# redwarp/kmeans-gpu

Hardware: AMD Instinct MI355X
Metric: pixels/sec per Lloyd iteration (8192x8192, k=256) (higher is better)
Workload: dtype f32; 1 GPU; synthetic uniform RGBA 8192x8192 (seed 0x5EED0003), k=256, one Lloyd iteration = update + assign (labels written every iteration) + accumulate; width=8192, height=8192, k=256, collective_backend=none (one rank), collective_ranks=1, label_pass=before the next iteration, update=by the last launch of the assign pass (kmg_lloyd_assign_update)

## Files before the change

### kmeans-gpu_amd/csrc/kmg_cube.hip

```cpp

#include "kmg_internal.h"
#include "kmg_table_dev.h"

#include <hip/hip_fp16.h>
#include <stdlib.h>

namespace kmg {

typedef float f32x2 __attribute__((ext_vector_type(2)));


namespace {

constexpr uint32_t kMaxListed = 32;
constexpr uint32_t kMaxLong = 256;
constexpr uint32_t kLongFlag = 0x200u;

__device__ __forceinline__ uint32_t sel3(uint32_t i, uint32_t x0, uint32_t x1, uint32_t x2)
{
    return i == 0u ? x0 : (i == 1u ? x1 : x2);
}

__device__ __forceinline__ int round_dir(int g, int m)
{
    const int a = g < 0 ? -g : g;
    const int r = (4 * a >= 3 * m ? 1 : 0) + (4 * a >= m ? 1 : 0);
    return g < 0 ? -r : r;
}

typedef unsigned short u16x2 __attribute__((ext_vector_type(2)));

__device__ __forceinline__ uint32_t group8_or(uint32_t v)
{
    v |= dpp_u32<kDppXor1>(v);
    v |= dpp_u32<kDppXor2>(v);
    v |= dpp_u32<kDppHalfMirror>(v);
    return v;
}

__device__ __forceinline__ uint32_t group8_min_u32(uint32_t v)
{
    v = min(v, dpp_u32<kDppXor1>(v));
    v = min(v, dpp_u32<kDppXor2>(v));
    v = min(v, dpp_u32<kDppHalfMirror>(v));
    return v;
}

__device__ __forceinline__ uint32_t group8_max_u32(uint32_t v)
{
    v = max(v, dpp_u32<kDppXor1>(v));
    v = max(v, dpp_u32<kDppXor2>(v));
    v = max(v, dpp_u32<kDppHalfMirror>(v));
    return v;
}



__device__ __forceinline__ uint32_t cell_pair_entry(const uint32_t idx[8], uint32_t occ, uint32_t lane)
{
    uint32_t rem = occ;
    uint32_t lab0 = 0, lab1 = 0, lab2 = 0, cnt0 = 0, cnt1 = 0, cnt2 = 0, msk0 = 0, msk1 = 0, msk2 = 0, n_occ = 0;
#pragma unroll
    for (int t = 0; t < 3; ++t) {
        const unsigned long long any = __ballot(rem != 0u);
        if (any) {
            uint32_t mine = 0;
#pragma unroll
            for (int q = 7; q >= 0; --q) mine = ((rem >> q) & 1u) ? idx[q] : mine;
            const uint32_t v = lane_value(mine, (uint32_t)__builtin_ctzll(any));
            uint32_t mm = 0;
#pragma unroll
            for (int q = 0; q < 8; ++q) mm |= (idx[q] == v ? 1u : 0u) << q;
            mm &= rem;
            rem &= ~mm;
            const uint32_t packed = wave_add_u32((uint32_t)__builtin_popcount(mm) | (t == 0 ? (uint32_t)__builtin_popcount(occ) << 10 : 0u));
            const uint32_t c = packed & 1023u;
            if (t == 0) { lab0 = v; msk0 = mm; cnt0 = c; n_occ = packed >> 10; }
            if (t == 1) { lab1 = v; msk1 = mm; cnt1 = c; }
            if (t == 2) { lab2 = v; msk2 = mm; cnt2 = c; }
        }
    }
    uint32_t a = 0;
    if (cnt1 > cnt0) a = 1;
    if (cnt2 > sel3(a, cnt0, cnt1, cnt2)) a = 2;
    uint32_t b = a == 0u ? 1u : 0u;
    if (a != 1u && b != 1u && cnt1 > sel3(b, cnt0, cnt1, cnt2)) b = 1;
    if (a != 2u && cnt2 > sel3(b, cnt0, cnt1, cnt2)) b = 2;
    const uint32_t labA = sel3(a, lab0, lab1, lab2), labB = sel3(b, lab0, lab1, lab2);
    const uint32_t mA = sel3(a, msk0, msk1, msk2), mB = sel3(b, msk0, msk1, msk2);
    const uint32_t rest = occ & ~mA;
    const uint32_t nA = sel3(a, cnt0, cnt1, cnt2), nR = n_occ - nA;
    if (nR == 0u) return pair_entry(labA, labA, 0u, 0u, 0u);

    const uint32_t half = ((lane >> 5) & 1u) | (((lane >> 4) & 1u) << 10) | (((lane >> 3) & 1u) << 20);
    const uint32_t hR = wave_add_u32((uint32_t)__builtin_popcount(rest) * half);
    const uint32_t hA = wave_add_u32((uint32_t)__builtin_popcount(mA) * half);
    const int gx = (int)((hR & 1023u) * nA) - (int)((hA & 1023u) * nR);
    const int gy = (int)(((hR >> 10) & 1023u) * nA) - (int)(((hA >> 10) & 1023u) * nR);
    const int gz = (int)((hR >> 20) * nA) - (int)((hA >> 20) * nR);
    const int ax = gx < 0 ? -gx : gx, ay = gy < 0 ? -gy : gy, az = gz < 0 ? -gz : gz;
    const int m = ax > ay ? (ax > az ? ax : az) : (ay > az ? ay : az);
    int nx = 2, ny = 0, nz = 0;
    if (m > 0) { nx = round_dir(gx, m); ny = round_dir(gy, m); nz = round_dir(gz, m); }

    const int xl = (int)(((lane >> 5) & 1u) * 4u + ((lane >> 1) & 3u));
    const int yl = (int)(((lane >> 4) & 1u) * 4u + (lane & 1u) * 2u);
    const int zl = (int)(((lane >> 3) & 1u) * 4u);
    const int bias = 7 * ((nx < 0 ? -nx : 0) + (ny < 0 ? -ny : 0) + (nz < 0 ? -nz : 0));
    const int p0 = nx * xl + ny * yl + nz * zl + bias;
    int p[8];
#pragma unroll
    for (int q = 0; q < 8; ++q) p[q] = p0 + ny * (q >> 2) + nz * (q & 3);
    const uint32_t notB = occ & ~mB;
    uint32_t tl = 63u, hi = 64u;
#pragma unroll
    for (int q = 0; q < 8; ++q) {
        if ((rest >> q) & 1u) tl = min(tl, (uint32_t)p[q]);
        if ((notB >> q) & 1u) hi = min(hi, (uint32_t)(63 - p[q]));
    }
    u16x2 packed = __builtin_bit_cast(u16x2, tl | (hi << 16));
    packed = __builtin_elementwise_min(packed, __builtin_bit_cast(u16x2, dpp_u32<kDppXor1>(__builtin_bit_cast(uint32_t, packed))));
    packed = __builtin_elementwise_min(packed, __builtin_bit_cast(u16x2, dpp_u32<kDppXor2>(__builtin_bit_cast(uint32_t, packed))));
    packed = __builtin_elementwise_min(packed, __builtin_bit_cast(u16x2, dpp_u32<kDppHalfMirror>(__builtin_bit_cast(uint32_t, packed))));
    packed = __builtin_elementwise_min(packed, __builtin_bit_cast(u16x2, dpp_u32<kDppMirror>(__builtin_bit_cast(uint32_t, packed))));
    packed = __builtin_elementwise_min(packed, __builtin_bit_cast(u16x2, (uint32_t)__builtin_amdgcn_update_dpp(-1, (int)__builtin_bit_cast(uint32_t, packed), 0x142, 0xA, 0xF, false)));
    packed = __builtin_elementwise_min(packed, __builtin_bit_cast(u16x2, (uint32_t)__builtin_amdgcn_update_dpp(-1, (int)__builtin_bit_cast(uint32_t, packed), 0x143, 0xC, 0xF, false)));
    const uint32_t pk = lane_value(__builtin_bit_cast(uint32_t, packed), 63);
    const int tlo = (int)(pk & 0xFFFFu);
    const int thi = 63 - (int)(pk >> 16);
    const int w = thi + 1 > tlo ? thi + 1 - tlo : 0;
    const uint32_t code = pair_dir_code(nx, ny, nz);
    if (w <= 6) return pair_entry(labA, labB, code, (uint32_t)tlo, (uint32_t)w);
    uint32_t low = 0, high = 0;
#pragma unroll
    for (int q = 0; q < 8; ++q) {
        if ((occ >> q) & 1u) { low += p[q] < tlo ? 1u : 0u; high += p[q] > thi ? 1u : 0u; }
    }
    const uint32_t lh = wave_add_u32(low | (high << 10));
    if ((lh & 1023u) >= (lh >> 10)) return pair_entry(labA, labB, code, (uint32_t)tlo, 7u);
    const int range = 7 * ((nx < 0 ? -nx : nx) + (ny < 0 ? -ny : ny) + (nz < 0 ? -nz : nz));
    return pair_entry(labB, labA, pair_dir_code(-nx, -ny, -nz), (uint32_t)(range - thi), 7u);
}

__device__ __forceinline__ uint32_t merge_state(uint32_t a, uint32_t b)
{
    return (a == kSubEmpty) ? b : ((b == kSubEmpty || b == a) ? a : (uint32_t)kSubMixed);
}

template <typename LabelT>
__device__ __forceinline__ void store_labels64(LabelT *dst64, uint32_t label, uint32_t lane)
{
    if (sizeof(LabelT) == 1) {
        const uint32_t t = label | (dpp_u32<kDppXor1>(label) << 8);
        const uint32_t u = t | (dpp_u32<kDppXor2>(t) << 16);
        if ((lane & 3u) == 0u) reinterpret_cast<uint32_t *>(dst64)[lane >> 2] = u;
    } else {
        const uint32_t t = label | (dpp_u32<kDppXor1>(label) << 16);
        if ((lane & 1u) == 0u) reinterpret_cast<uint32_t *>(dst64)[lane >> 1] = t;
    }
}


struct alignas(16) CellWork {
    uint16_t list[kMaxListed];
    unsigned long long br[4];
    uint32_t npop;
    uint32_t scan_set;
    uint32_t pad[6];
};
static_assert(sizeof(CellWork) == 128, "CellWork layout");

constexpr uint32_t kPairPending = 0xFFFFFFFEu;

constexpr uint32_t kLongSegs = 16, kLongSegCap = kCells / kLongSegs, kLongCount = 0, kLongCells = 64;
constexpr size_t kListsWords = kLongCells + kCells;
constexpr uint32_t kItemCands = 12;

__device__ __forceinline__ void flush_bins(const unsigned long long *bins, uint32_t k, uint32_t repl, uint32_t bin_stride,
                                           int64_t *sums, uint32_t n_rows)
{
    __syncthreads();
    unsigned long long *row = reinterpret_cast<unsigned long long *>(sums) + (uint64_t)(blockIdx.x % n_rows) * 4ull * k;
    for (uint32_t i = threadIdx.x; i < 4u * k; i += blockDim.x) {
        unsigned long long v = 0ull;
        for (uint32_t r = 0; r < repl; ++r) v += bins[(uint64_t)r * bin_stride + i];
        if (v) atomicAdd(row + i, v);
    }
}

// ... 1106 lines not shown
            const uint32_t ps = __builtin_amdgcn_readfirstlane((uint32_t)s_pend[pi]);
            const uint32_t pcell = __builtin_amdgcn_readfirstlane(s_cell[ps]);
            const uint2 lv = *reinterpret_cast<const uint2 *>(s_lbl + ps * kCellColours + lane * 8u);
            uint32_t e = kPairPending;
            if (!(flags & kCubeNoEntries)) {
                const uint32_t round = (pi - wv) / kSmallWaves;
                const uint32_t occ = round == 0u ? occ_early[0] : (round == 1u ? occ_early[1] :
                                     (occ_bits ? (uint32_t)occ_bits[(uint64_t)pcell * 64u + lane] : 0xFFu));
                uint32_t idx[8];
#pragma unroll
                for (uint32_t q = 0; q < 4u; ++q) { idx[q] = (lv.x >> (8u * q)) & 0xFFu; idx[4u + q] = (lv.y >> (8u * q)) & 0xFFu; }
                e = cell_pair_entry(idx, occ, lane);
            }
            if (lane == 0u) pair_entries[pcell] = e;
            *reinterpret_cast<uint2 *>(colour_labels + (uint64_t)pcell * kCellColours + lane * 8u) = lv;
        }
        __syncthreads();
        if (threadIdx.x < 2u) s_count[threadIdx.x] = 0u;
        if (threadIdx.x == 3u) s_count[3] = 0u;
        __syncthreads();
    }
    if (stats && lane == 0u) {
        atomicAdd(stats + 0, st_single); atomicAdd(stats + 1, st_multi); atomicAdd(stats + 2, st_decided);
        atomicAdd(stats + 3, st_scanned); atomicAdd(stats + 4, st_cands);
    }
    if (SUMS) {
        __syncthreads();
        unsigned long long *row = reinterpret_cast<unsigned long long *>(sums) + (uint64_t)(blockIdx.x % n_rows) * 4ull * k;
        for (uint32_t i = threadIdx.x; i < 4u * k; i += kSmallBlock) {
            unsigned long long v = 0ull;
            for (uint32_t r = 0; r < kSmallRepl; ++r) v += bins[(uint64_t)r * bin_stride + i];
            if (v) atomicAdd(row + i, v);
        }
    }
}

constexpr int kOneBlock = 1024;
constexpr uint32_t kOneWaves = kOneBlock / 64, kOneCells = kOneWaves * 8u;
constexpr uint32_t kOneItems = kOneCells * 4u;
constexpr uint32_t kOneTests = 384;
constexpr uint32_t kOneRepl = 4;

constexpr uint32_t kOneTaskSlots = (kCells / kOneCells) * kOneWaves;
constexpr uint32_t kOneBalWords = 80;
size_t cube_balance_bytes() { return sizeof(uint16_t) * 4u * kOneTaskSlots; }

static size_t cube_one_lds_bytes(uint32_t k, bool with_sums)
{
    const size_t bins = with_sums ? sizeof(unsigned long long) * kOneRepl * (4ull * k + 4ull) : 0u;
    return sizeof(float4) * 256u + bins + (size_t)kOneCells * kCellColours + sizeof(uint4) * kOneItems + sizeof(uint16_t) * kOneWaves * kOneTests +
           sizeof(unsigned long long) * kOneCells * 4u + sizeof(uint32_t) * kOneBlock * 2u + (size_t)kOneCells * 64u +
           sizeof(uint32_t) * kOneCells * 3u + sizeof(uint32_t) * (8u + kOneWaves + kOneBalWords) + sizeof(uint16_t) * kOneCells * kMaxListed;
}

#ifdef KMG_TOOLS
__device__ unsigned long long g_one_stamps[(kCells / kOneCells) * 12u];
#define KMG_STAMP(i) do { if (threadIdx.x == 0u) g_one_stamps[blockIdx.x * 12u + (i)] = wall_clock64(); } while (0)
#define KMG_STAMP_VALUE(i, v) do { if (threadIdx.x == 0u) g_one_stamps[blockIdx.x * 12u + (i)] = (v); } while (0)
#else
#define KMG_STAMP(i) do { } while (0)
#define KMG_STAMP_VALUE(i, v) do { } while (0)
#endif

template <bool SUMS>
__global__ __launch_bounds__(kOneBlock) __attribute__((amdgpu_waves_per_eu(4, 4))) void k_cube_one(
    const uint32_t *__restrict__ hist, const int64_t *__restrict__ agg, const int64_t *__restrict__ sub_agg,
    const uint8_t *__restrict__ occ_bits, const uint32_t *__restrict__ work, const CellBounds *__restrict__ bounds,
    const CellBounds *__restrict__ sub_bounds, const float *__restrict__ sub_affine, const Centroid *__restrict__ cent, uint32_t k,
    const float4 *__restrict__ lab_table, uint64_t *__restrict__ masks_out, uint8_t *__restrict__ colour_labels,
    uint16_t *__restrict__ sub_table, int64_t *__restrict__ sums, uint32_t n_rows, uint32_t flags,
    unsigned long long *__restrict__ stats, uint16_t *__restrict__ bal_state, uint32_t bal_pass)
{
    extern __shared__ float4 smem4[];
    float4 *s_cent = smem4;
    unsigned long long *bins = reinterpret_cast<unsigned long long *>(smem4 + 256);
    const uint32_t bin_stride = 4u * k + 4u;
    const uint32_t n_bins = SUMS ? kOneRepl * bin_stride : 0u;
    uint8_t *s_lbl = reinterpret_cast<uint8_t *>(bins + n_bins);
    uint4 *s_item = reinterpret_cast<uint4 *>(s_lbl + kOneCells * kCellColours);
    uint16_t *s_test = reinterpret_cast<uint16_t *>(s_item + kOneItems);
    unsigned long long *s_cmask = reinterpret_cast<unsigned long long *>(s_test + kOneWaves * kOneTests);
    uint32_t *s_mask = reinterpret_cast<uint32_t *>(s_cmask + kOneCells * 4u);
    uint32_t *s_ref = s_mask + kOneBlock;
    uint8_t *s_occ = reinterpret_cast<uint8_t *>(s_ref + kOneBlock);
    uint32_t *s_cell = reinterpret_cast<uint32_t *>(s_occ + kOneCells * 64u);
    uint32_t *s_npop = s_cell + kOneCells;
    uint32_t *s_left = s_npop + kOneCells;
    uint32_t *s_count = s_left + kOneCells;
    uint32_t *s_bal = s_count + 8 + kOneWaves;
    uint16_t *s_list = reinterpret_cast<uint16_t *>(s_bal + kOneBalWords);

    const uint32_t vz = opaque_vgpr_zero();
    const uint32_t n_work_v = SUMS ? work[vz] : kCells;
    if (threadIdx.x < 256u) {
        float4 v = make_float4(1.0e18f, 0.0f, 0.0f, 0.0f);
        if (threadIdx.x < k) { const Centroid c = cent[threadIdx.x]; v = make_float4(c.L, c.a, c.b, c.C); }
        s_cent[threadIdx.x] = v;
    }
    if (threadIdx.x < 8u + kOneWaves) s_count[threadIdx.x] = 0u;
    if (SUMS) for (uint32_t i = threadIdx.x; i < n_bins; i += kOneBlock) bins[i] = 0ull;
    if (bal_state && (threadIdx.x >> 6) == kOneWaves - 1u) {
        const uint32_t bl = threadIdx.x & 63u;
        const uint32_t nw = __builtin_amdgcn_readfirstlane(n_work_v);
        const uint32_t bcpw = min(8u, max(1u, (nw + gridDim.x * kOneWaves - 1u) / (gridDim.x * kOneWaves)));
        const uint32_t btasks = (nw + bcpw - 1u) / bcpw, bused = (btasks + gridDim.x - 1u) / gridDim.x;
        uint16_t *cur = bal_state + (bal_pass & 1u) * 2u * kOneTaskSlots;
        const uint16_t *prev = bal_state + ((bal_pass + 1u) & 1u) * 2u * kOneTaskSlots;
        uint32_t id = 0xFFFFu;
        if (bal_pass == 0u) {
            if (bl < bused && blockIdx.x * bused + bl < btasks) id = blockIdx.x * bused + bl;
        } else {
            const uint32_t partner = blockIdx.x ^ (1u << ((bal_pass - 1u) & 7u));
            const uint32_t lo_wg = min(blockIdx.x, partner), hi_wg = max(blockIdx.x, partner);
            const uint32_t src = ((bl & 16u) ? hi_wg : lo_wg) * kOneWaves + (bl & 15u);
            uint32_t e_id = 0xFFFFu, e_w = 0u;
            if (bl < 32u) { e_id = prev[src]; e_w = prev[kOneTaskSlots + src]; }
            if (e_id >= btasks) { e_id = 0xFFFFu; e_w = 0u; }
            if (bl < 32u) s_bal[bl] = (e_w << 16) | e_id;
            __builtin_amdgcn_wave_barrier();
            uint32_t rank = 0;
            for (uint32_t j = 0; j < 32u; ++j) {
                const uint32_t ow = s_bal[j] >> 16;
                rank += (ow > e_w || (ow == e_w && j < bl)) ? 1u : 0u;
            }
            if (bl < 32u) s_bal[32u + rank] = (e_w << 16) | e_id;
            __builtin_amdgcn_wave_barrier();
            const uint32_t sorted = bl < 32u ? s_bal[32u + bl] : 0u;
            const bool i_am_hi = blockIdx.x == hi_wg;
            uint32_t t0 = 0, t1 = 0, c0 = 0, c1 = 0;
#pragma unroll
            for (uint32_t r = 0; r < 32u; ++r) {
                const uint32_t e = lane_value(sorted, r);
                const bool to_hi = c0 >= kOneWaves || (c1 < kOneWaves && t1 < t0);
                if (to_hi) { if (i_am_hi && bl == c1) id = e & 0xFFFFu; ++c1; t1 += e >> 16; }
                else       { if (!i_am_hi && bl == c0) id = e & 0xFFFFu; ++c0; t0 += e >> 16; }
            }
        }
        if (bl < kOneWaves) { cur[blockIdx.x * kOneWaves + bl] = (uint16_t)id; s_bal[64u + bl] = id; }
    }
    __syncthreads();
    if (threadIdx.x < k) {
        const float4 c = s_cent[threadIdx.x];
        if (!(fabsf(c.x) <= 1024.0f && fabsf(c.y) <= 1024.0f && fabsf(c.z) <= 1024.0f)) s_count[2] = 1u;
    }
    __syncthreads();
    const bool dominance = sub_affine != nullptr && s_count[2] == 0u;

    const uint32_t lane = threadIdx.x & 63u, wv = threadIdx.x >> 6;
    const uint32_t ci = lane >> 3, sub = lane & 7u, slot = wv * 8u + ci;
    unsigned long long *my_bins = bins + (uint64_t)(lane & (kOneRepl - 1u)) * bin_stride;
    uint32_t *pair_entries = reinterpret_cast<uint32_t *>(sub_table + kSubCells + kCells);
    const uint32_t words = (k + 63u) / 64u;
    unsigned long long st_single = 0, st_multi = 0, st_unlisted = 0, st_decided = 0, st_scanned = 0, st_cands = 0, st_removed = 0, st_one = 0;
    float4 c4[4];
#pragma unroll
    for (int w = 0; w < 4; ++w) c4[w] = s_cent[w * 64 + lane];

    const uint32_t n_work = __builtin_amdgcn_readfirstlane(n_work_v);
    const uint32_t cpw = min(8u, max(1u, (n_work + gridDim.x * kOneWaves - 1u) / (gridDim.x * kOneWaves)));
    const uint32_t tasks = (n_work + cpw - 1u) / cpw;
    const uint32_t waves_used = (tasks + gridDim.x - 1u) / gridDim.x;
    if (!bal_state && blockIdx.x * waves_used >= tasks) return;
    {
        KMG_STAMP(0);
        uint32_t task = wv < waves_used ? blockIdx.x * waves_used + wv : tasks;
        if (bal_state) task = min(s_bal[64u + wv], tasks);
        const uint32_t prime = tasks % 2053u ? 2053u : 1031u;
        const uint32_t pos = (uint32_t)(((uint64_t)task * prime) % tasks) + ci * tasks;
        const bool valid = task < tasks && ci < cpw && pos < n_work;
        const uint32_t cell = valid ? ((SUMS && n_work != kCells) ? work[1u + pos] : pos) : 0u;
        const uint32_t sc = cell * 8u + sub;
        const uint32_t cell_a = (uint32_t)__builtin_amdgcn_ds_bpermute((int)(((lane >> 4) * 8u) << 2), (int)cell);
        const uint32_t cell_b = (uint32_t)__builtin_amdgcn_ds_bpermute((int)(((4u + (lane >> 4)) * 8u) << 2), (int)cell);
        const float cbv_a = reinterpret_cast<const float *>(bounds + cell_a)[lane & 15u];
        const float cbv_b = reinterpret_cast<const float *>(bounds + cell_b)[lane & 15u];
        const float4 *sbp = reinterpret_cast<const float4 *>(sub_bounds + sc);
        const float4 sb0 = sbp[0], sb1 = sbp[1], sb2 = sbp[2];
        longlong2 g01 = {0, 0}, g23 = {0, 1};
        long long cell_sum = 0;
        if (SUMS) {
            const longlong2 *sp = reinterpret_cast<const longlong2 *>(sub_agg + (uint64_t)sc * 4u);
            g01 = sp[0]; g23 = sp[1];
            cell_sum = agg[4ull * cell + (sub & 3u)];
        }
        uint2 occ8 = make_uint2(0xFFFFFFFFu, 0xFFFFFFFFu);
        if (occ_bits) occ8 = *reinterpret_cast<const uint2 *>(occ_bits + (uint64_t)cell * 64u + sub * 8u);
        if (sub == 0u) s_cell[slot] = cell;

        float *s_cb = reinterpret_cast<float *>(s_lbl + (size_t)wv * 8u * kCellColours);
        s_cb[lane] = cbv_a;
        s_cb[64u + lane] = cbv_b;
        __builtin_amdgcn_wave_barrier();
        for (uint32_t c = 0; c < cpw; ++c) {
            const uint32_t ccell = lane_value(cell, c * 8u);
            const bool cvalid = lane_value((uint32_t)valid, c * 8u) != 0u;
            const float4 *cq = reinterpret_cast<const float4 *>(s_cb + c * 16u);
            const float4 q0 = cq[0], q1 = cq[1], q2 = cq[2];
            CellBounds cb;
            cb.L0 = q0.x; cb.L1 = q0.y; cb.a0 = q0.z; cb.a1 = q0.w;
            cb.b0 = q1.x; cb.b1 = q1.y; cb.C0 = q1.z; cb.C1 = q1.w;
            cb.wC0 = q2.x; cb.wC1 = q2.y; cb.wH0 = q2.z; cb.wH1 = q2.w;
            float lo[4], U = 3.0e38f;
#pragma unroll
            for (int w = 0; w < 4; ++w) {
                const KeyRange r = key_range(cb, c4[w].x, c4[w].y, c4[w].z, c4[w].w);
                lo[w] = r.lo;
                U = fminf(U, r.hi);
            }
            const float Us = mask_threshold(wave_min(U));
            unsigned long long mw[4];
            uint32_t npop = 0, first = 0;
#pragma unroll
            for (uint32_t w = 0; w < 4u; ++w) {
                mw[w] = __ballot(w * 64u + lane < k && lo[w] <= Us);
                if (npop == 0u && mw[w]) first = w * 64u + (uint32_t)__builtin_ctzll(mw[w]);
                npop += (uint32_t)__builtin_popcountll(mw[w]);
            }
            const uint32_t cslot = wv * 8u + c;
            if (cvalid && lane < words) masks_out[(uint64_t)ccell * words + lane] = lane == 0u ? mw[0] : (lane == 1u ? mw[1] : (lane == 2u ? mw[2] : mw[3]));
            if (lane == 0u) s_npop[cslot] = npop | (first << 16);
            if (npop > 1u && npop <= kMaxListed) {
                uint32_t at = 0;
#pragma unroll
                for (uint32_t w = 0; w < 4u; ++w) {
                    if ((mw[w] >> lane) & 1ull) s_list[cslot * kMaxListed + at + bits_below_lane(mw[w])] = (uint16_t)(w * 64u + lane);
                    at += (uint32_t)__builtin_popcountll(mw[w]);
                }
            } else if (npop > kMaxListed) {
                if (lane < 4u) s_cmask[cslot * 4u + lane] = lane == 0u ? mw[0] : (lane == 1u ? mw[1] : (lane == 2u ? mw[2] : mw[3]));
            }
        }
        __builtin_amdgcn_wave_barrier();
        KMG_STAMP(1);

        const uint32_t np_first = s_npop[slot];
        const uint32_t npop = valid ? (np_first & 0xFFFFu) : 1u, first = np_first >> 16;
        const bool listed = valid && npop > 1u && npop <= kMaxListed;
        const bool unlisted = valid && npop > kMaxListed;
        const bool occupied = valid && (SUMS ? g23.y != 0 : true);
        uint32_t sm = 0u, istar = 0u, ubits = 0u;
        if (listed) {
            CellBounds sb;
            sb.L0 = sb0.x; sb.L1 = sb0.y; sb.a0 = sb0.z; sb.a1 = sb0.w;
            sb.b0 = sb1.x; sb.b1 = sb1.y; sb.C0 = sb1.z; sb.C1 = sb1.w;
            sb.wC0 = sb2.x; sb.wC1 = sb2.y; sb.wH0 = sb2.z; sb.wH1 = sb2.w;
            uint32_t Ubest = 0x7F7FFFE0u;
            for (uint32_t p = 0; p < npop; ++p) {
                const float4 c = s_cent[s_list[slot * kMaxListed + p]];
                Ubest = min(Ubest, ((float_to_bits(key_range(sb, c.x, c.y, c.z, c.w).hi) + 31u) & ~31u) | p);
            }
            const float Us = mask_threshold(bits_to_float(Ubest & ~31u));
            for (uint32_t p = 0; p < npop; ++p) {
                const float4 c = s_cent[s_list[slot * kMaxListed + p]];
                sm |= (key_range(sb, c.x, c.y, c.z, c.w).lo <= Us ? 1u : 0u) << p;
            }
            istar = Ubest & 31u;
            ubits = Ubest & ~31u;
        }
        const uint32_t np0 = (uint32_t)__builtin_popcount(sm);
        const bool was_decided = listed && occupied && np0 == 1u;
        const bool mine = listed && occupied && np0 > 1u;
        s_mask[threadIdx.x] = sm;
        *reinterpret_cast<uint2 *>(s_occ + slot * 64u + sub * 8u) = occ8;
        const uint32_t others = (mine && dominance) ? sm & ~(1u << istar) : 0u;
        if (others) {
            s_ref[threadIdx.x] = ubits | istar;
            const uint32_t nt = (uint32_t)__builtin_popcount(others);
            uint32_t at = atomicAdd(&s_count[8u + wv], nt);
            for (uint32_t m = others; m && at < kOneTests; m &= m - 1u, ++at)
                s_test[wv * kOneTests + at] = (uint16_t)((lane << 5) | (uint32_t)__builtin_ctz(m));
        }
        KMG_STAMP(2);
        __builtin_amdgcn_fence(__ATOMIC_RELEASE, "workgroup");
        __builtin_amdgcn_wave_barrier();
        __builtin_amdgcn_fence(__ATOMIC_ACQUIRE, "workgroup");
        if (dominance) {
            const uint32_t n_tests = min(__builtin_amdgcn_readfirstlane(s_count[8u + wv]), kOneTests);
            for (uint32_t t = lane; t < n_tests; t += 64u) {
                const uint32_t ent = (uint32_t)s_test[wv * kOneTests + t];
                const uint32_t e = wv * 64u + (ent >> 5), tp = ent & 31u;
                const uint32_t r = s_ref[e];
                const float4 cj = s_cent[s_list[(e >> 3) * kMaxListed + tp]], ci4 = s_cent[s_list[(e >> 3) * kMaxListed + (r & 31u)]];
                HalfModel mdl;
                mdl.load(sub_affine, (uint64_t)s_cell[e >> 3] * 8u + (e & 7u));
                if (dominated(mdl, cj, ci4, bits_to_float(r & ~31u))) atomicAnd(&s_mask[e], ~(1u << tp));
            }
            __builtin_amdgcn_fence(__ATOMIC_RELEASE, "workgroup");
            __builtin_amdgcn_wave_barrier();
            __builtin_amdgcn_fence(__ATOMIC_ACQUIRE, "workgroup");
        }
        KMG_STAMP(3);

        const uint32_t nm = s_mask[threadIdx.x];
        const uint32_t np = (uint32_t)__builtin_popcount(nm);
        const bool one = mine && np == 1u, still = mine && np > 1u;
        const uint32_t X = listed ? (uint32_t)s_list[slot * kMaxListed + (nm ? (uint32_t)__builtin_ctz(nm) : 0u)] : first;
        const bool open = still || (unlisted && occupied);
        const uint32_t scan8 = group8_or(open ? 1u << sub : 0u);
        const bool settled = one || was_decided;
        const uint32_t xmin = group8_min_u32(settled ? X : 255u), xmax = group8_max_u32(settled ? X : 0u);
        const bool single = valid && npop == 1u;
        const bool uniform = single || (listed && scan8 == 0u && xmin == xmax);
        const uint32_t Xu = single ? first : xmin;
        if (SUMS) {
            if (uniform) {
                if (sub < 4u) atomicAdd(my_bins + 4ull * Xu + sub, (unsigned long long)cell_sum);
            } else if (settled) {
                unsigned long long *to = my_bins + 4ull * X;
                atomicAdd(to + 0, (unsigned long long)g01.x); atomicAdd(to + 1, (unsigned long long)g01.y);
                atomicAdd(to + 2, (unsigned long long)g23.x); atomicAdd(to + 3, (unsigned long long)g23.y);
            }
        }
        {
            const uint32_t x4 = (settled ? X : 0u) * 0x01010101u;
            const uint4 xv = make_uint4(x4, x4, x4, x4);
            if (uniform) {
                if (sub == 0u) pair_entries[cell] = pair_entry(Xu, Xu, 0u, 0u, 0u);
                if (flags & 1u) {
                    const uint32_t m4 = Xu * 0x01010101u;
                    uint4 *dst = reinterpret_cast<uint4 *>(colour_labels + (uint64_t)cell * kCellColours + sub * 64u);
                    dst[0] = dst[1] = dst[2] = dst[3] = make_uint4(m4, m4, m4, m4);
                }
            } else if (valid) {
                uint4 *dst = reinterpret_cast<uint4 *>(s_lbl + slot * kCellColours + sub * 64u);
                dst[0] = xv; dst[1] = xv; dst[2] = xv; dst[3] = xv;
            }
        }
        unsigned long long pend0_b = 0ull;
        {
            const uint32_t rank = (uint32_t)__builtin_popcount(scan8 & ((1u << sub) - 1u));
            const bool head = open && (rank & 1u) == 0u;
            const uint32_t after = scan8 & ~((2u << sub) - 1u);
            const uint32_t s1 = after ? (uint32_t)__builtin_ctz(after) : 8u;
            const uint32_t un = listed ? (nm | ((head && s1 < 8u) ? s_mask[threadIdx.x - sub + s1] : 0u)) : 0u;
            const uint32_t n_un = (uint32_t)__builtin_popcount(un);
            const uint32_t type = unlisted ? 2u : (n_un > kItemCands ? 1u : 0u);
            const bool pend = valid && !uniform && sub == 0u;
            if (pend) s_left[slot] = ((uint32_t)__builtin_popcount(scan8) + 1u) >> 1;
            pend0_b = __ballot(pend && scan8 == 0u);
            const unsigned long long item_b = __ballot(head);
            if (bal_state) {
                const uint32_t cost = wave_add_u32(head ? 4u + (type == 2u ? npop : n_un) : 0u);
                if (lane == 0u) bal_state[(bal_pass & 1u) * 2u * kOneTaskSlots + kOneTaskSlots + blockIdx.x * kOneWaves + wv] = (uint16_t)min(cost, 65535u);
            }
            uint32_t i_base = 0u;
            if (lane == 0u && item_b) i_base = atomicAdd(&s_count[0], (uint32_t)__builtin_popcountll(item_b));
            i_base = __builtin_amdgcn_readfirstlane(i_base);
            if (head) {
                uint32_t iw0 = un, iw1 = 0u, iw2 = 0u;
                if (type == 0u) {
                    iw0 = 0u;
                    uint32_t q = 0u;
                    for (uint32_t m = un; m; m &= m - 1u, ++q) {
                        const uint32_t cc = (uint32_t)s_list[slot * kMaxListed + (uint32_t)__builtin_ctz(m)] << (8u * (q & 3u));
                        iw0 |= q < 4u ? cc : 0u; iw1 |= (q >= 4u && q < 8u) ? cc : 0u; iw2 |= q >= 8u ? cc : 0u;
                    }
                }
                s_item[i_base + bits_below_lane(item_b)] = make_uint4(slot | (sub << 7) | (s1 << 10) | (n_un << 14) | (type << 30), iw0, iw1, iw2);
            }
            if (stats) {
                st_single += (uint32_t)__builtin_popcountll(__ballot(single && sub == 0u));
                st_multi += (uint32_t)__builtin_popcountll(__ballot(valid && !single && sub == 0u));
                st_unlisted += (uint32_t)__builtin_popcountll(__ballot(unlisted && sub == 0u));
                st_decided += (uint32_t)__builtin_popcountll(__ballot(was_decided));
                st_scanned += (uint32_t)__builtin_popcountll(__ballot(mine || (unlisted && occupied)));
                st_cands += wave_add_u32(mine ? np0 : ((unlisted && occupied) ? npop : 0u));
                st_removed += wave_add_u32((uint32_t)__builtin_popcount(sm & ~nm));
                st_one += (uint32_t)__builtin_popcountll(__ballot(one));
            }
        }
        KMG_STAMP(4);
        __syncthreads();
        const uint32_t n_items = s_count[0];
        KMG_STAMP_VALUE(8, n_items); KMG_STAMP_VALUE(10, s_count[8]);

        auto cell_entry = [&](const uint32_t ps) {
            const uint32_t pcell = __builtin_amdgcn_readfirstlane(s_cell[ps]);
            const uint2 lv = *reinterpret_cast<const uint2 *>(s_lbl + ps * kCellColours + lane * 8u);
            uint32_t e = kPairPending;
            if (!(flags & kCubeNoEntries)) {
                const uint32_t occ = (uint32_t)s_occ[ps * 64u + lane];
                uint32_t idx[8];
// ... 325 lines not shown
```

Before: 307.6 billion pixels/s.

## Evaluate cell candidate masks per 8-lane group instead of looping cells per wave

Replaces the serial per-cell loop, in which the whole wave scanned all 256 centroids for one cell at a time, with a layout where each 8-lane group handles its own cell and each lane scores 32 centroids from LDS using a skewed addressing pattern. Candidate masks, popcounts, first index and list offsets are then built with 8-lane DPP reductions and a prefix scan. This removes the cpw-long serial loop and the wave-wide ballots. In exchange it adds more registers per lane (32 lo values), extra LDS centroid reads, and per-lane list writes.

New measurement: 315.2 billion pixels/s (median of 6 runs). 2.5% higher.

```diff
diff --git a/kmeans-gpu_amd/csrc/kmg_cube.hip b/kmeans-gpu_amd/csrc/kmg_cube.hip
--- a/kmeans-gpu_amd/csrc/kmg_cube.hip
+++ b/kmeans-gpu_amd/csrc/kmg_cube.hip
@@ -35,6 +35,14 @@
     v |= dpp_u32<kDppXor1>(v);
     v |= dpp_u32<kDppXor2>(v);
     v |= dpp_u32<kDppHalfMirror>(v);
+    return v;
+}
+
+__device__ __forceinline__ uint32_t group8_add_u32(uint32_t v)
+{
+    v += dpp_u32<kDppXor1>(v);
+    v += dpp_u32<kDppXor2>(v);
+    v += dpp_u32<kDppHalfMirror>(v);
     return v;
 }
 
@@ -1447,9 +1455,6 @@
     uint32_t *pair_entries = reinterpret_cast<uint32_t *>(sub_table + kSubCells + kCells);
     const uint32_t words = (k + 63u) / 64u;
     unsigned long long st_single = 0, st_multi = 0, st_unlisted = 0, st_decided = 0, st_scanned = 0, st_cands = 0, st_removed = 0, st_one = 0;
-    float4 c4[4];
-#pragma unroll
-    for (int w = 0; w < 4; ++w) c4[w] = s_cent[w * 64 + lane];
 
     const uint32_t n_work = __builtin_amdgcn_readfirstlane(n_work_v);
     const uint32_t cpw = min(8u, max(1u, (n_work + gridDim.x * kOneWaves - 1u) / (gridDim.x * kOneWaves)));
@@ -1486,43 +1491,54 @@
         s_cb[lane] = cbv_a;
         s_cb[64u + lane] = cbv_b;
         __builtin_amdgcn_wave_barrier();
-        for (uint32_t c = 0; c < cpw; ++c) {
-            const uint32_t ccell = lane_value(cell, c * 8u);
-            const bool cvalid = lane_value((uint32_t)valid, c * 8u) != 0u;
-            const float4 *cq = reinterpret_cast<const float4 *>(s_cb + c * 16u);
+        {
+            const float4 *cq = reinterpret_cast<const float4 *>(s_cb + ci * 16u);
             const float4 q0 = cq[0], q1 = cq[1], q2 = cq[2];
             CellBounds cb;
             cb.L0 = q0.x; cb.L1 = q0.y; cb.a0 = q0.z; cb.a1 = q0.w;
             cb.b0 = q1.x; cb.b1 = q1.y; cb.C0 = q1.z; cb.C1 = q1.w;
             cb.wC0 = q2.x; cb.wC1 = q2.y; cb.wH0 = q2.z; cb.wH1 = q2.w;
-            float lo[4], U = 3.0e38f;
-#pragma unroll
-            for (int w = 0; w < 4; ++w) {
-                const KeyRange r = key_range(cb, c4[w].x, c4[w].y, c4[w].z, c4[w].w);
-                lo[w] = r.lo;
-                U = fminf(U, r.hi);
-            }
-            const float Us = mask_threshold(wave_min(U));
-            unsigned long long mw[4];
-            uint32_t npop = 0, first = 0;
-#pragma unroll
-            for (uint32_t w = 0; w < 4u; ++w) {
-                mw[w] = __ballot(w * 64u + lane < k && lo[w] <= Us);
-                if (npop == 0u && mw[w]) first = w * 64u + (uint32_t)__builtin_ctzll(mw[w]);
-                npop += (uint32_t)__builtin_popcountll(mw[w]);
-            }
-            const uint32_t cslot = wv * 8u + c;
-            if (cvalid && lane < words) masks_out[(uint64_t)ccell * words + lane] = lane == 0u ? mw[0] : (lane == 1u ? mw[1] : (lane == 2u ? mw[2] : mw[3]));
-            if (lane == 0u) s_npop[cslot] = npop | (first << 16);
-            if (npop > 1u && npop <= kMaxListed) {
-                uint32_t at = 0;
-#pragma unroll
-                for (uint32_t w = 0; w < 4u; ++w) {
-                    if ((mw[w] >> lane) & 1ull) s_list[cslot * kMaxListed + at + bits_below_lane(mw[w])] = (uint16_t)(w * 64u + lane);
-                    at += (uint32_t)__builtin_popcountll(mw[w]);
-                }
-            } else if (npop > kMaxListed) {
-                if (lane < 4u) s_cmask[cslot * 4u + lane] = lane == 0u ? mw[0] : (lane == 1u ? mw[1] : (lane == 2u ? mw[2] : mw[3]));
+            const float4 *p0 = s_cent + 33u * sub, *p1 = p0 - 32;
+            auto centroid_of_step = [&](uint32_t i) { return i < 25u ? p0[i] : (i + sub >= 32u ? p1 : p0)[i]; };
+            float lo[32], U = 3.0e38f;
+            float4 cn[4];
+#pragma unroll
+            for (uint32_t q = 0; q < 4u; ++q) cn[q] = centroid_of_step(q);
+#pragma unroll
+            for (uint32_t i0 = 0; i0 < 32u; i0 += 4u) {
+                float4 cc[4];
+#pragma unroll
+                for (uint32_t q = 0; q < 4u; ++q) { cc[q] = cn[q]; if (i0 + 4u < 32u) cn[q] = centroid_of_step(i0 + 4u + q); }
+#pragma unroll
+                for (uint32_t q = 0; q < 4u; ++q) {
+                    const KeyRange r = key_range(cb, cc[q].x, cc[q].y, cc[q].z, cc[q].w);
+                    lo[i0 + q] = r.lo;
+                    U = fminf(U, r.hi);
+                    asm volatile("" : "+v"(lo[i0 + q]));
+                }
+                __builtin_amdgcn_sched_barrier(0);
+            }
+            const float Us = mask_threshold(group8_min(U));
+            uint32_t turned = 0u;
+#pragma unroll
+            for (uint32_t i = 0; i < 32u; ++i) turned |= (lo[i] <= Us ? 1u : 0u) << i;
+            const uint32_t j0 = 32u * sub;
+            const uint32_t in_k = j0 >= k ? 0u : (k - j0 >= 32u ? 0xFFFFFFFFu : (1u << (k - j0)) - 1u);
+            const uint32_t word = __builtin_rotateleft32(turned, sub) & in_k;
+            const uint32_t pc = (uint32_t)__builtin_popcount(word);
+            const uint32_t cnpop = group8_add_u32(pc);
+            const uint32_t low = group8_min_u32(word ? j0 + (uint32_t)__builtin_ctz(word) : 0xFFFFu);
+            const uint32_t cfirst = cnpop ? low : 0u;
+            const uint32_t t1 = dpp_u32<0x111>(pc), u1 = pc + (t1 & (sub >= 1u ? 0xFFFFFFFFu : 0u));
+            const uint32_t t2 = dpp_u32<0x112>(u1), u2 = u1 + (t2 & (sub >= 2u ? 0xFFFFFFFFu : 0u));
+            const uint32_t t4 = dpp_u32<0x114>(u2), upto = u2 + (t4 & (sub >= 4u ? 0xFFFFFFFFu : 0u));
+            if (valid && sub < 2u * words) reinterpret_cast<uint32_t *>(masks_out)[(uint64_t)cell * (2u * words) + sub] = word;
+            if (sub == 0u) s_npop[slot] = cnpop | (cfirst << 16);
+            if (cnpop > 1u && cnpop <= kMaxListed) {
+                uint32_t at = slot * kMaxListed + upto - pc;
+                for (uint32_t m = word; m; m &= m - 1u) s_list[at++] = (uint16_t)(j0 + (uint32_t)__builtin_ctz(m));
+            } else if (cnpop > kMaxListed) {
+                reinterpret_cast<uint32_t *>(s_cmask)[slot * 8u + sub] = word;
             }
         }
         __builtin_amdgcn_wave_barrier();
```
